# IlzeAmandaA/VAE-GP-ODE

Measured on AMD Instinct MI355X. Metric: latent_trajectories_per_sec, higher is better.
Workload: dtype f32; 1 GPU; configs[1]: ode1 DF q=6 M=100 S=256 T=16 batch=256; step = full ELBO training step (encoder, GP draw, rk4 rollout, decoder, ELBO, backward, Adam), L=1; global_batch=256, mc_draws=1, solver=rk4 (3/8 rule), parallelism=dp1, hip_graph=True, graph_scope=whole, gp_side_stream=True, batchnorm=per-process statistics

## Files before the change

vae-gp-ode_amd/csrc/conv_bwd_v2.hpp:

```cpp
#pragma once
#include "conv_mfma.hpp"

namespace gp {

template <class L> struct BdV2 {
  using PL = BwdDataPolicy<L, L::CI>;
  static constexpr int KC = L::CO, NC = L::CI, KK = L::K * L::K;
  static constexpr int NCT = NC / 16;
  static constexpr int NKS = KK * (KC / 4);
  static constexpr int NPX = L::HI * L::HI;
  static constexpr int SRC = KC * L::HO * L::HO;
  static constexpr int PS = PL::PS, HP = PL::HP, IMG = KC * PS;
  static constexpr int NBUF = 3, NCW = 8, NTHR = 768, NLT = NTHR - 64 * NCW;
  static constexpr int TPW = 2;
  static constexpr int WIN = 16 * 4 * TPW;
  static constexpr int PF = 2;
  static_assert(NCT * 4 == NCW, "the two consumers of a SIMD split the output channels");
  static_assert(KC % 4 == 0 && L::HO % 4 == 0 && SRC % 4 == 0, "float4 rows of the source");
  static_assert(WIN <= NPX, "a window touches at most two images");
  static constexpr int koff(int s) { return (s / (KC / 4)) / L::K * HP + (s / (KC / 4)) % L::K + (s % (KC / 4)) * 4 * PS; }
  static_assert(4 * koff(NKS - 1) < 65536, "operand offsets fit the ds_read immediate");
  static constexpr size_t lds_bytes() { return sizeof(float) * (size_t)NBUF * IMG; }
};

template <class E, int NT>
__device__ __forceinline__ void bdv2_tiles(const float* __restrict__ s_buf, const int (&base)[E::TPW], const float (&wr)[E::NKS],
                                           f32x4 (&acc)[E::TPW]) {
  float bf[E::PF + 1][NT];
  auto fetch = [&](auto sc) {
    constexpr int s = decltype(sc)::value;
#pragma unroll
    for (int t = 0; t < NT; ++t) bf[s % (E::PF + 1)][t] = s_buf[base[t] + E::koff(s)];
  };
#pragma unroll
  for (int t = 0; t < NT; ++t) acc[t] = f32x4{0.f, 0.f, 0.f, 0.f};
  static_for<E::PF>([&](auto sc) { fetch(sc); });
  static_for<E::NKS>([&](auto sc) {
    constexpr int s = decltype(sc)::value;
    if constexpr (s + E::PF < E::NKS) fetch(std::integral_constant<int, s + E::PF>{});
    __builtin_amdgcn_sched_barrier(0);
#pragma unroll
    for (int t = 0; t < NT; ++t) acc[t] = __builtin_amdgcn_mfma_f32_16x16x4f32(wr[s], bf[s % (E::PF + 1)][t], acc[t], 0, 0, 0);
    __builtin_amdgcn_sched_barrier(0);
  });
}

template <class L>
__global__ __launch_bounds__(768) void k_conv_bwd_data_v2(const float* __restrict__ gy, const float* __restrict__ w, float* __restrict__ gx,
                                                          int B) {
  using E = BdV2<L>;
  using PL = typename E::PL;
  constexpr int KC = E::KC, NC = E::NC, KK = E::KK, NPX = E::NPX, IMG = E::IMG, PS = E::PS, HP = E::HP, WIN = E::WIN, NKS = E::NKS;
  constexpr int HO = L::HO, P = L::P, NLT = E::NLT;
  float* s_buf = igemm_smem;
  const int tid = threadIdx.x, lane = tid & 63, wave = __builtin_amdgcn_readfirstlane(tid >> 6);
  const int nit = ((int)blockIdx.x < B) ? (B - 1 - (int)blockIdx.x) / (int)gridDim.x + 1 : 0;
  const int npx = nit * NPX, nwin = (npx + WIN - 1) / WIN;
  auto last_img = [&](int i) { return min(nit - 1, (i * WIN + WIN - 1) / NPX); };

  for (int e = tid; e < E::NBUF * IMG / 4; e += E::NTHR) reinterpret_cast<float4*>(s_buf)[e] = float4{0.f, 0.f, 0.f, 0.f};
  __syncthreads();

  if (wave >= E::NCW) {
    __builtin_amdgcn_s_setprio(3);
    const int lt = tid - 64 * E::NCW;
    constexpr int N4 = E::SRC / 4, NLD = (N4 + NLT - 1) / NLT;
    auto stage = [&](int j) __attribute__((always_inline)) {
      const float4* src = reinterpret_cast<const float4*>(gy) + (size_t)((int)blockIdx.x + j * (int)gridDim.x) * N4;
      float* buf = s_buf + (j % E::NBUF) * IMG;
      float4 v[NLD];
#pragma unroll
      for (int i = 0; i < NLD; ++i) v[i] = src[min(lt + NLT * i, N4 - 1)];
#pragma unroll
      for (int i = 0; i < NLD; ++i) {
        const int f = lt + NLT * i;
        const int pl = (4 * f) / (HO * HO), q = (4 * f) % (HO * HO), row = q / HO, col = q % HO;
        float* d = buf + pl * PS + (row + P) * HP + col + P;
        if (f < N4) { d[0] = v[i].x; d[1] = v[i].y; d[2] = v[i].z; d[3] = v[i].w; }
      }
    };
    if (nit > 0) stage(0);
    __syncthreads();
    for (int i = 0; i < nwin; ++i) {
      if (i + 1 < nwin && last_img(i + 1) > last_img(i)) stage(last_img(i + 1));
      __syncthreads();
    }
    return;
  }

  const int lr = lane & 15, lk = lane >> 4, ct = wave >> 2, sm = wave & 3;
  float wr[NKS];
#pragma unroll
  for (int s = 0; s < NKS; ++s) wr[s] = w[((size_t)(16 * ct + lr) * KC + 4 * (s % (KC / 4)) + lk) * KK + s / (KC / 4)];
  __syncthreads();
  for (int i = 0; i < nwin; ++i) {
    const int t0 = i * WIN + 16 * sm;
    int base[E::TPW], mm[E::TPW];
#pragma unroll
    for (int t = 0; t < E::TPW; ++t) {
      mm[t] = t0 + 64 * t + lr;
      const int m = min(mm[t], npx - 1);
      const int j = m / NPX, p = m - j * NPX;
      base[t] = (j % E::NBUF) * IMG + lk * PS + PL::template C<0>::pix_addr(p);
    }
    f32x4 acc[E::TPW];
    int nt = 0;
    if (t0 + 64 < npx) { bdv2_tiles<E, 2>(s_buf, base, wr, acc); nt = 2; }
    else if (t0 < npx) { bdv2_tiles<E, 1>(s_buf, base, wr, acc); nt = 1; }
#pragma unroll
    for (int t = 0; t < E::TPW; ++t) {
      if (t < nt && mm[t] < npx) {
        const int j = mm[t] / NPX, p = mm[t] - j * NPX;
        float* o = gx + ((size_t)((int)blockIdx.x + j * (int)gridDim.x) * NC + 16 * ct + 4 * lk) * NPX + p;
#pragma unroll
        for (int r = 0; r < 4; ++r) o[(size_t)r * NPX] = acc[t][r];
      }
    }
    __syncthreads();
  }
}

}
```

vae-gp-ode_amd/csrc/vae_conv_tiled.hip:

```cpp
#include <hip/hip_runtime.h>
#include <cstdlib>
#include <cstdint>
#include "gp_launch.hpp"
#include <type_traits>
#include "conv_layers.hpp"
#include "conv_mfma.hpp"
#include "conv_dec10_mfma.hpp"
#include "conv_dec1_mfma.hpp"
#include "conv_dec4_mfma.hpp"

namespace gp {



extern __shared__ __attribute__((aligned(16))) float tsm[];

template <class L, int IPB>
__global__ __launch_bounds__(256) void k_convT_fwd(const float* __restrict__ x, const float* __restrict__ w,
                                                    const float* __restrict__ bias, float* __restrict__ y, int B) {
  constexpr int CI = L::CI, CO = L::CO, HI = L::HI, HO = L::HO, HP = L::HP, K = L::K, S = L::S, P = L::P, PL = L::PL;
  constexpr int CPT = CO % 16 == 0 ? 16 : 8;
  static_assert(CO % CPT == 0, "8 or 16 output channels per thread");
  constexpr int NG = CO / CPT;
  constexpr int IMG = CI * HP * HP;
  float* s_img = tsm;
  float* s_w = tsm + IPB * IMG;
  const int tid = threadIdx.x;
  const int b0 = blockIdx.x * IPB;
  const int nimg = min(IPB, B - b0);
  for (int e = tid; e < IPB * IMG; e += 256) {
    const int im = e / IMG, r = e % IMG, ci = r / (HP * HP), yy = (r / HP) % HP - PL, xx = r % HP - PL;
    float v = 0.f;
    if (im < nimg && yy >= 0 && yy < HI && xx >= 0 && xx < HI) v = x[(((size_t)(b0 + im) * CI + ci) * HI + yy) * HI + xx];
    s_img[e] = v;
  }
  for (int cls = 0; cls < S * S; ++cls) {
    const int py = cls / S, px = cls % S;
    const int nty = (K - py + S - 1) / S, ntx = (K - px + S - 1) / S;
    __syncthreads();
    for (int e = tid; e < nty * ntx * CI * CO; e += 256) {
      const int co = e % CO, ci = (e / CO) % CI, tap = e / (CO * CI);
      const int ky = py + S * (tap / ntx), kx = px + S * (tap % ntx);
      s_w[e] = w[(((size_t)ci * CO + co) * K + ky) * K + kx];
    }
    __syncthreads();
    const int qy0 = (P - py + S - 1 > 0) ? (P - py + S - 1) / S : 0, qx0 = (P - px + S - 1 > 0) ? (P - px + S - 1) / S : 0;
    const int ny = (HO - 1 + P - py) / S - qy0 + 1, nx = (HO - 1 + P - px) / S - qx0 + 1;
    const int items = nimg * ny * nx * NG;
    for (int it = tid; it < items; it += 256) {
      const int g = it % NG, p = (it / NG) % (ny * nx), im = it / (NG * ny * nx);
      const int qy = qy0 + p / nx, qx = qx0 + p % nx;
      float acc[CPT];
#pragma unroll
      for (int c = 0; c < CPT; ++c) acc[c] = bias ? bias[g * CPT + c] : 0.f;
      const float* img = s_img + im * IMG;
      for (int ty = 0; ty < nty; ++ty) {
        for (int tx = 0; tx < ntx; ++tx) {
          const float* ip = img + (qy - ty + PL) * HP + (qx - tx + PL);
          const float4* wp = reinterpret_cast<const float4*>(s_w + ((ty * ntx + tx) * CI) * CO + g * CPT);
#pragma unroll 4
          for (int ci = 0; ci < CI; ++ci) {
            const float v = ip[ci * HP * HP];
#pragma unroll
            for (int q = 0; q < CPT / 4; ++q) {
              const float4 wq = wp[ci * (CO / 4) + q];
              acc[4 * q] = fmaf(v, wq.x, acc[4 * q]); acc[4 * q + 1] = fmaf(v, wq.y, acc[4 * q + 1]);
              acc[4 * q + 2] = fmaf(v, wq.z, acc[4 * q + 2]); acc[4 * q + 3] = fmaf(v, wq.w, acc[4 * q + 3]);
            }
          }
        }
      }
      const int oy = S * qy + py - P, ox = S * qx + px - P;
      float* yp = y + (((size_t)(b0 + im) * CO + g * CPT) * HO + oy) * HO + ox;
#pragma unroll
      for (int c = 0; c < CPT; ++c) yp[(size_t)c * HO * HO] = acc[c];
    }
  }
}


template <class L, int IPB, int COC>
__global__ __launch_bounds__(256) void k_convT_bwd_data(const float* __restrict__ gy, const float* __restrict__ w,
                                                         float* __restrict__ gx, int B) {
  constexpr int CI = L::CI, CO = L::CO, HI = L::HI, HO = L::HO, GPD = L::GP_, K = L::K, S = L::S, P = L::P, KK = K * K;
  static_assert(CI % 16 == 0 && CO % COC == 0, "blocking");
  constexpr int NG = CI / 16;
  constexpr int IMG = CO * GPD * GPD;
  float* s_img = tsm;
  float* s_w = tsm + IPB * IMG;
  const int tid = threadIdx.x;
  const int b0 = blockIdx.x * IPB;
  const int nimg = min(IPB, B - b0);
  for (int e = tid; e < IPB * IMG; e += 256) {
    const int im = e / IMG, r = e % IMG, co = r / (GPD * GPD), yy = (r / GPD) % GPD - P, xx = r % GPD - P;
    float v = 0.f;
    if (im < nimg && yy >= 0 && yy < HO && xx >= 0 && xx < HO) v = gy[(((size_t)(b0 + im) * CO + co) * HO + yy) * HO + xx];
    s_img[e] = v;
  }
  const int items = nimg * HI * HI * NG;
  constexpr int MAXIT = (IPB * HI * HI * NG + 255) / 256;
  float acc[MAXIT][16];
#pragma unroll
  for (int r = 0; r < MAXIT; ++r)
#pragma unroll
    for (int c = 0; c < 16; ++c) acc[r][c] = 0.f;
  for (int c0 = 0; c0 < CO; c0 += COC) {
    __syncthreads();
    for (int e = tid; e < COC * KK * CI; e += 256) {
      const int ci = e % CI, tap = (e / CI) % KK, co = c0 + e / (CI * KK);
      s_w[e] = w[((size_t)ci * CO + co) * KK + tap];
    }
    __syncthreads();
#pragma unroll
    for (int r = 0; r < MAXIT; ++r) {
      const int it = tid + 256 * r;
      if (it < items) {
        const int g = it % NG, p = (it / NG) % (HI * HI), im = it / (NG * HI * HI);
        const int iy = p / HI, ix = p % HI;
        const float* img = s_img + im * IMG + (c0 * GPD + S * iy) * GPD + S * ix;
        for (int co = 0; co < COC; ++co) {
#pragma unroll
          for (int ky = 0; ky < K; ++ky) {
#pragma unroll
            for (int kx = 0; kx < K; ++kx) {
              const float v = img[(co * GPD + ky) * GPD + kx];
              const float4* wp = reinterpret_cast<const float4*>(s_w + ((co * KK + ky * K + kx) * CI) + g * 16);
              const float4 w0 = wp[0], w1 = wp[1], w2 = wp[2], w3 = wp[3];
              float* a = acc[r];
              a[0] = fmaf(v, w0.x, a[0]); a[1] = fmaf(v, w0.y, a[1]); a[2] = fmaf(v, w0.z, a[2]); a[3] = fmaf(v, w0.w, a[3]);
              a[4] = fmaf(v, w1.x, a[4]); a[5] = fmaf(v, w1.y, a[5]); a[6] = fmaf(v, w1.z, a[6]); a[7] = fmaf(v, w1.w, a[7]);
              a[8] = fmaf(v, w2.x, a[8]); a[9] = fmaf(v, w2.y, a[9]); a[10] = fmaf(v, w2.z, a[10]); a[11] = fmaf(v, w2.w, a[11]);
              a[12] = fmaf(v, w3.x, a[12]); a[13] = fmaf(v, w3.y, a[13]); a[14] = fmaf(v, w3.z, a[14]); a[15] = fmaf(v, w3.w, a[15]);
            }
          }
        }
      }
    }
  }
#pragma unroll
  for (int r = 0; r < MAXIT; ++r) {
    const int it = tid + 256 * r;
    if (it < items) {
      const int g = it % NG, p = (it / NG) % (HI * HI), im = it / (NG * HI * HI);
      float* gp = gx + (((size_t)(b0 + im) * CI + g * 16) * HI * HI) + p;
#pragma unroll
      for (int c = 0; c < 16; ++c) gp[(size_t)c * HI * HI] = acc[r][c];
    }
  }
}

template <class L, int COW>
__global__ __launch_bounds__(256) void k_convT_wgrad(const float* __restrict__ x, const float* __restrict__ gy,
                                                      float* __restrict__ part, int B, int b_per_split) {
  constexpr int CI = L::CI, CO = L::CO, HI = L::HI, HO = L::HO, GPD = L::GP_, K = L::K, S = L::S, P = L::P, KK = K * K;
  constexpr int NQ = COW / 4;
  constexpr int NT = CI * NQ;
  constexpr int PSPLIT = 256 / NT;
  static_assert(NT <= 256 && 256 % NT == 0, "thread mapping");
  float* s_x = tsm;
  float* s_g = tsm + HI * HI * CI;
  const int tid = threadIdx.x;
  const int ci = tid % CI, q = (tid / CI) % NQ, ps = tid / NT;
  const int co0 = blockIdx.y * COW;
  const int b0 = blockIdx.x * b_per_split, b1 = min(B, b0 + b_per_split);
  float acc[KK][4];
#pragma unroll
  for (int t = 0; t < KK; ++t) { acc[t][0] = 0.f; acc[t][1] = 0.f; acc[t][2] = 0.f; acc[t][3] = 0.f; }
  for (int b = b0; b < b1; ++b) {
    __syncthreads();
    for (int e = tid; e < HI * HI * CI; e += 256) {
      const int c = e % CI, p = e / CI;
      s_x[e] = x[((size_t)b * CI + c) * HI * HI + p];
    }
    for (int e = tid; e < GPD * GPD * COW; e += 256) {
      const int c = e % COW, xx = (e / COW) % GPD - P, yy = e / (COW * GPD) - P;
      float v = 0.f;
      if (yy >= 0 && yy < HO && xx >= 0 && xx < HO) v = gy[(((size_t)b * CO + co0 + c) * HO + yy) * HO + xx];
      s_g[e] = v;
    }
    __syncthreads();
    for (int p = ps; p < HI * HI; p += PSPLIT) {
      const int iy = p / HI, ix = p % HI;
      const float xv = s_x[p * CI + ci];
      const float* gp = s_g + ((S * iy) * GPD + S * ix) * COW + q * 4;
#pragma unroll
      for (int ky = 0; ky < K; ++ky) {
#pragma unroll
        for (int kx = 0; kx < K; ++kx) {
          const float4 g4 = *reinterpret_cast<const float4*>(gp + (ky * GPD + kx) * COW);
          float* a = acc[ky * K + kx];
          a[0] = fmaf(xv, g4.x, a[0]); a[1] = fmaf(xv, g4.y, a[1]); a[2] = fmaf(xv, g4.z, a[2]); a[3] = fmaf(xv, g4.w, a[3]);
        }
      }
    }
  }
  __syncthreads();
  float* s_red = tsm;
  if (PSPLIT > 1) {
#pragma unroll
    for (int t = 0; t < KK; ++t)
#pragma unroll
      for (int c = 0; c < 4; ++c) s_red[((size_t)ps * NT + (tid % NT)) * (KK * 4) + t * 4 + c] = acc[t][c];
    __syncthreads();
  }
  if (ps == 0) {
    float* out = part + (size_t)blockIdx.x * CI * CO * KK;
#pragma unroll
    for (int t = 0; t < KK; ++t)
#pragma unroll
      for (int c = 0; c < 4; ++c) {
        float v = acc[t][c];
        if (PSPLIT > 1)
          for (int sp = 1; sp < PSPLIT; ++sp) v += s_red[((size_t)sp * NT + (tid % NT)) * (KK * 4) + t * 4 + c];
        out[((size_t)ci * CO + co0 + q * 4 + c) * KK + t] = v;
      }
  }
}


template <int IPB>
__global__ __launch_bounds__(256) void k_dec10_fwd(const float* __restrict__ x, const float* __restrict__ w,
                                                    const float* __restrict__ bias, float* __restrict__ y, int B) {
  constexpr int CI = 16, H = 28, WP = 32, IMG = CI * WP * WP;
  float* s_img = tsm;
  float* s_w = tsm + IPB * IMG;
  const int tid = threadIdx.x;
  const int b0 = blockIdx.x * IPB;
  const int nimg = min(IPB, B - b0);
  for (int e = tid; e < IPB * IMG; e += 256) {
    const int im = e / IMG, r = e % IMG, ci = r / (WP * WP), yy = (r / WP) % WP - 2, xx = r % WP - 2;
    float v = 0.f;
    if (im < nimg && yy >= 0 && yy < H && xx >= 0 && xx < H) v = x[(((size_t)(b0 + im) * CI + ci) * H + yy) * H + xx];
    s_img[e] = v;
  }
  for (int e = tid; e < CI * 5 * 8; e += 256) {
    const int kx = e % 8, ky = (e / 8) % 5, ci = e / 40;
    s_w[e] = kx < 5 ? w[(size_t)ci * 25 + ky * 5 + kx] : 0.f;
  }
  __syncthreads();
  const float bv = bias ? bias[0] : 0.f;
  const int items = nimg * H * 7;
  for (int it = tid; it < items; it += 256) {
    const int seg = it % 7, oy = (it / 7) % H, im = it / (7 * H);
    const int ox0 = seg * 4;
    float acc[4] = {bv, bv, bv, bv};
    const float* img = s_img + im * IMG;
#pragma unroll 2
    for (int ci = 0; ci < CI; ++ci) {
#pragma unroll
      for (int ky = 0; ky < 5; ++ky) {
        const float4* rp = reinterpret_cast<const float4*>(img + (ci * WP + (oy + 4 - ky)) * WP + ox0);
        const float4 a = rp[0], b = rp[1];
        const float v[8] = {a.x, a.y, a.z, a.w, b.x, b.y, b.z, b.w};
        const float4 w4 = *reinterpret_cast<const float4*>(s_w + (ci * 5 + ky) * 8);
        const float w5 = s_w[(ci * 5 + ky) * 8 + 4];
        const float wk[5] = {w4.x, w4.y, w4.z, w4.w, w5};
#pragma unroll
        for (int j = 0; j < 4; ++j)
#pragma unroll
          for (int kx = 0; kx < 5; ++kx) acc[j] = fmaf(v[j + 4 - kx], wk[kx], acc[j]);
      }
    }
    *reinterpret_cast<float4*>(y + ((size_t)(b0 + im) * H + oy) * H + ox0) = make_float4(acc[0], acc[1], acc[2], acc[3]);
  }
}

__global__ __launch_bounds__(256) void k_dec10_wgrad(const float* __restrict__ x, const float* __restrict__ gy,
                                                      float* __restrict__ part, int B, int b_per_split) {
  constexpr int CI = 16, H = 28, NP = H * H, XS = NP + 1, GW = 32;
  float* s_x = tsm;
  float* s_g = tsm + CI * XS;
  const int tid = threadIdx.x, ci = tid & 15, pl = tid >> 4;
  const int b0 = blockIdx.x * b_per_split, b1 = min(B, b0 + b_per_split);
  float acc[25];
#pragma unroll
  for (int t = 0; t < 25; ++t) acc[t] = 0.f;
  for (int b = b0; b < b1; ++b) {
    __syncthreads();
    for (int e = tid; e < CI * NP; e += 256) s_x[(e / NP) * XS + e % NP] = x[(size_t)b * CI * NP + e];
    for (int e = tid; e < GW * GW; e += 256) {
      const int yy = e / GW - 2, xx = e % GW - 2;
      s_g[e] = (yy >= 0 && yy < H && xx >= 0 && xx < H) ? gy[(size_t)b * NP + yy * H + xx] : 0.f;
    }
    __syncthreads();
    for (int p = pl; p < NP; p += 16) {
      const int iy = p / H, ix = p % H;
      const float xv = s_x[ci * XS + p];
      const float* gp = s_g + iy * GW + ix;
#pragma unroll
      for (int ky = 0; ky < 5; ++ky)
#pragma unroll
        for (int kx = 0; kx < 5; ++kx) acc[ky * 5 + kx] = fmaf(xv, gp[ky * GW + kx], acc[ky * 5 + kx]);
    }
  }
  __syncthreads();
  float* s_red = tsm;
#pragma unroll
  for (int t = 0; t < 25; ++t) s_red[(pl * 16 + ci) * 25 + t] = acc[t];
  __syncthreads();
  for (int e = tid; e < CI * 25; e += 256) {
    float v = 0.f;
    for (int l = 0; l < 16; ++l) v += s_red[l * 400 + e];
    part[(size_t)blockIdx.x * 400 + e] = v;
  }
}

__global__ void k_sum_splits_t(const float* __restrict__ part, int nsplit, size_t n, float* __restrict__ out) {
  const size_t e = (size_t)blockIdx.x * blockDim.x + threadIdx.x;
  if (e >= n) return;
  float acc = 0.f;
  for (int s = 0; s < nsplit; ++s) acc += part[(size_t)s * n + e];
  out[e] = acc;
}

template <class L> static bool matches(int Ci_conv, int Co_conv, int H, int Ho, int K, int S, int P) {
  return Ci_conv == L::CO && Co_conv == L::CI && H == L::HO && Ho == L::HI && K == L::K && S == L::S && P == L::P;
}

static bool use_mfma() {
  static int v = -1;
  if (v < 0) { const char* e = getenv("GPODE_CONV_VALU"); v = (e && e[0] == '1') ? 0 : 1; }
  return v == 1;
}

constexpr int kSinkMaxWg = 512;

template <class PL, int IPB, int TG, int NCJ, bool PAIR = false, int NTHR = 512, bool DB = false, bool STATS = false>
static int launch_igemm(const float* x, const float* w, const float* bias, float* y, int B, hipStream_t st, const char* what,
                        const float* in_bn = nullptr, const BnSink* sink = nullptr) {
  constexpr size_t lds = igemm_lds_bytes<PL, IPB, DB, STATS>();
  static_assert(lds <= (NTHR >= 512 ? 160 : 80) * 1024, "LDS budget");
  auto km = k_conv_igemm<PL, IPB, TG, NCJ, PAIR, NTHR, DB, STATS>;
  if (set_max_lds((const void*)km, lds)) return 1;
  const int ngroups = (B + IPB - 1) / IPB;
  const int cap = num_cus() * (NTHR >= 512 ? 1 : 2);
  if (STATS && cap > kSinkMaxWg) return set_error("%s: more workgroups than the statistics scratch holds", what);
  hipLaunchKernelGGL(km, ngroups < cap ? ngroups : cap, NTHR, lds, st, x, w, bias, y, B, in_bn, STATS ? *sink : BnSink{});
  return check_launch(what);
}

template <class L, int IPB, int IPBM, int COS>
static int launch_T1(const float* x, const float* w, const float* bias, float* y, int B, hipStream_t st, const float* in_bn,
                     const BnSink* sink = nullptr) {
  constexpr int MAXTAPS = ((L::K + L::S - 1) / L::S) * ((L::K + L::S - 1) / L::S);
  const size_t lds = sizeof(float) * ((size_t)IPB * L::CI * L::HP * L::HP + (size_t)MAXTAPS * L::CI * L::CO);
  if (use_mfma() && (reinterpret_cast<uintptr_t>(x) & 15) == 0) {
    constexpr int TG = COS >= 64 ? 1 : (COS >= 32 ? 2 : 4);
    constexpr bool PAIR = L::S == 2 && (L::HO % 2 == 0) && (L::P % 2 == 1);
    if constexpr (std::is_same<L, Dec7>::value) {
      static const bool db = [] { const char* e = getenv("GPODE_DEC7_FWD_DB"); return e && e[0] == '1'; }();
      if (db) return launch_igemm<FwdPolicy<L, COS>, 1, TG, COS / 16, PAIR, 512, true>(x, w, bias, y, B, st, "convT_fwd_mfma", in_bn);
    }
    if (sink) return launch_igemm<FwdPolicy<L, COS>, IPBM, TG, COS / 16, PAIR, 512, false, true>(x, w, bias, y, B, st, "convT_fwd_mfma_stats", in_bn, sink);
    return launch_igemm<FwdPolicy<L, COS>, IPBM, TG, COS / 16, PAIR>(x, w, bias, y, B, st, "convT_fwd_mfma", in_bn);
  }
  if (sink) return set_error("convT forward with output statistics needs the matrix-core path (16-byte aligned input, GPODE_CONV_VALU unset)");
  if (in_bn) return set_error("convT forward with a fused BatchNorm input needs the matrix-core path (16-byte aligned input, GPODE_CONV_VALU unset)");
  auto kern = k_convT_fwd<L, IPB>;
  if (set_max_lds((const void*)kern, lds)) return 1;
  hipLaunchKernelGGL(kern, (B + IPB - 1) / IPB, 256, lds, st, x, w, bias, y, B);
  return check_launch("convT_fwd_tiled");
}

template <class L, int IPB, int COC, int IPBM, int CIS, int TG, int NCJ, int NTHR = 512>
static int launch_T2(const float* gy, const float* w, float* gx, int B, hipStream_t st) {
  if constexpr (IPBM > 0) {
    if (use_mfma() && (reinterpret_cast<uintptr_t>(gy) & 15) == 0)
      return launch_igemm<BwdDataPolicy<L, CIS>, IPBM, TG, NCJ, false, NTHR>(gy, w, nullptr, gx, B, st, "convT_bwd_data_mfma");
  }
  const size_t lds = sizeof(float) * ((size_t)IPB * L::CO * L::GP_ * L::GP_ + (size_t)COC * L::K * L::K * L::CI);
  auto kern = k_convT_bwd_data<L, IPB, COC>;
  if (set_max_lds((const void*)kern, lds)) return 1;
  hipLaunchKernelGGL(kern, (B + IPB - 1) / IPB, 256, lds, st, gy, w, gx, B);
  return check_launch("convT_bwd_data_tiled");
}

template <class L, int IPBM, int WM, int WN, int WT, bool PIPE>
static int launch_wgrad_mfma(const float* x, const float* gy, float* gw, float* scratch, int B, hipStream_t st, const float* in_bn) {
  constexpr int NTHR = WM * WN * WT * 64;
  constexpr size_t ldsm = wgrad_lds_bytes<L, IPBM>();
  static_assert(ldsm <= (NTHR == 512 ? 160 : 80) * 1024, "LDS budget");
  auto km = k_convT_wgrad_mfma<L, IPBM, WM, WN, WT, PIPE, false, NTHR>;
  auto kb = k_convT_wgrad_mfma<L, IPBM, WM, WN, WT, PIPE, true, NTHR>;
  if (set_max_lds((const void*)km, ldsm) || set_max_lds((const void*)kb, ldsm)) return 1;
  const int ngroups = (B + IPBM - 1) / IPBM;
  const int cap = num_cus() * (512 / NTHR);
  const int nwg = ngroups < cap ? ngroups : cap;
  if (in_bn) hipLaunchKernelGGL(kb, nwg, NTHR, ldsm, st, x, gy, scratch, B, in_bn);
  else hipLaunchKernelGGL(km, nwg, NTHR, ldsm, st, x, gy, scratch, B, in_bn);
  const size_t n = (size_t)L::CI * L::CO * L::K * L::K;
  if (reduce_job(RedJob{scratch, gw, nwg, (int)n, 1, L::CI / 16, L::CO / 16, L::K * L::K}, st)) return 1;
  return check_launch("convT_wgrad_mfma");
}

int wgrad_v2_dec7(const float* x, const float* gy, float* gw, float* scratch, int B, hipStream_t st, const float* in_bn);
int wgrad_v2_dec4(const float* x, const float* gy, float* gw, float* scratch, int B, hipStream_t st, const float* in_bn);
static bool wgrad_v2_enabled() {
  static const bool off = [] { const char* e = getenv("GPODE_WGRAD_V1"); return e && e[0] == '1'; }();
  return !off && use_mfma();
}

template <class L, int COW, int IPBM, int WM, int WN, int WT, bool PIPE>
static int launch_T3(const float* x, const float* gy, float* gw, float* scratch, int B, hipStream_t st, const float* in_bn) {
  if (use_mfma() && ((reinterpret_cast<uintptr_t>(x) | reinterpret_cast<uintptr_t>(gy)) & 15) == 0)
    return launch_wgrad_mfma<L, IPBM, WM, WN, WT, PIPE>(x, gy, gw, scratch, B, st, in_bn);
  if (in_bn) return set_error("convT weight gradient with a fused BatchNorm input needs the matrix-core path");
  constexpr int NT = L::CI * (COW / 4), PSPLIT = 256 / NT, KK = L::K * L::K;
  size_t fl = (size_t)L::HI * L::HI * L::CI + (size_t)L::GP_ * L::GP_ * COW;
  const size_t red = PSPLIT > 1 ? (size_t)PSPLIT * NT * KK * 4 : 0;
  if (red > fl) fl = red;
  const size_t lds = sizeof(float) * fl;
  int nsplit = B < 256 ? B : 256;
  const int bps = (B + nsplit - 1) / nsplit;
  nsplit = (B + bps - 1) / bps;
  auto kern = k_convT_wgrad<L, COW>;
  if (set_max_lds((const void*)kern, lds)) return 1;
  hipLaunchKernelGGL(kern, dim3(nsplit, L::CO / COW), 256, lds, st, x, gy, scratch, B, bps);
  const size_t n = (size_t)L::CI * L::CO * KK;
  if (reduce_job(RedJob{scratch, gw, nsplit, (int)n, 0, 0, 0, 0}, st)) return 1;
  return check_launch("convT_wgrad_tiled");
}


int tiled_bwd_data(const float* gy, const float* w, const float* bias, float* gx, int B, int Ci, int H, int W, int Co, int K, int S,
                   int P, int Ho, int Wo, const float* in_bn, hipStream_t st, const BnSink* sink) {
  if (H != W || Ho != Wo) return -1;
  if (sink && !(use_mfma() && (matches<Dec7>(Ci, Co, H, Ho, K, S, P) || matches<Dec4>(Ci, Co, H, Ho, K, S, P) ||
                               (matches<Dec1>(Ci, Co, H, Ho, K, S, P) && !in_bn))))
    return set_error("gpode_convT_fwd_stats: no specialisation for this geometry");
  if (matches<Dec7>(Ci, Co, H, Ho, K, S, P)) return launch_T1<Dec7, 3, 2, 16>(gy, w, bias, gx, B, st, in_bn, sink);
  if (matches<Dec4>(Ci, Co, H, Ho, K, S, P)) {
    static const int tapcols = [] { const char* e = getenv("GPODE_DEC4_TAPCOLS"); return e ? (e[0] == '1' ? 1 : 0) : -1; }();
    if ((tapcols == 1 || (tapcols < 0 && B <= 4 * num_cus())) && use_mfma()) {
      const size_t lds = sizeof(float) * (dec4::NPI * dec4::TLD + 4 * dec4::CI + (sink ? 2 * dec4::CO * dec4::NPO : 0));
      if (set_max_lds((const void*)dec4::k_fwd<true>, lds) || set_max_lds((const void*)dec4::k_fwd<false>, lds) ||
          set_max_lds((const void*)dec4::k_fwd<true, true>, lds) || set_max_lds((const void*)dec4::k_fwd<false, true>, lds)) return 1;
      const int nwg = B < num_cus() ? B : num_cus();
      const BnSink sk = sink ? *sink : BnSink{};
      if (sink && in_bn) hipLaunchKernelGGL((dec4::k_fwd<true, true>), nwg, 512, lds, st, gy, w, bias, gx, B, in_bn, sk);
      else if (sink) hipLaunchKernelGGL((dec4::k_fwd<false, true>), nwg, 512, lds, st, gy, w, bias, gx, B, in_bn, sk);
      else if (in_bn) hipLaunchKernelGGL((dec4::k_fwd<true>), nwg, 512, lds, st, gy, w, bias, gx, B, in_bn, sk);
      else hipLaunchKernelGGL((dec4::k_fwd<false>), nwg, 512, lds, st, gy, w, bias, gx, B, in_bn, sk);
      return check_launch("dec4_fwd_tapcols");
    }
    return launch_T1<Dec4, 3, 2, 16>(gy, w, bias, gx, B, st, in_bn, sink);
  }
  if (matches<Dec1>(Ci, Co, H, Ho, K, S, P)) {
    static const bool old = [] { const char* e = getenv("GPODE_DEC1_ENGINE"); return e && e[0] == '1'; }();
    if (!in_bn && use_mfma() && (!old || sink)) {
      const size_t lds = sizeof(float) * 2 * dec1::NPI * dec1::TLD;
      if (set_max_lds((const void*)dec1::k_fwd<false>, lds) || set_max_lds((const void*)dec1::k_fwd<true>, lds)) return 1;
      const int cap = 2 * num_cus();
      if (sink) hipLaunchKernelGGL(dec1::k_fwd<true>, B < cap ? B : cap, 256, lds, st, gy, w, bias, gx, B, *sink);
      else hipLaunchKernelGGL(dec1::k_fwd<false>, B < cap ? B : cap, 256, lds, st, gy, w, bias, gx, B, BnSink{});
      return check_launch("dec1_fwd_mfma");
    }
    return launch_T1<Dec1, 8, 8, 64>(gy, w, bias, gx, B, st, in_bn);
  }
  if (matches<Enc3>(Ci, Co, H, Ho, K, S, P) && !in_bn && B >= 96) {
    constexpr int IPB = 2;
    constexpr int MAXTAPS = ((Enc3::K + Enc3::S - 1) / Enc3::S) * ((Enc3::K + Enc3::S - 1) / Enc3::S);
    const size_t lds = sizeof(float) * ((size_t)IPB * Enc3::CI * Enc3::HP * Enc3::HP + (size_t)MAXTAPS * Enc3::CI * Enc3::CO);
    auto kern = k_convT_fwd<Enc3, IPB>;
    if (set_max_lds((const void*)kern, lds)) return 1;
    hipLaunchKernelGGL(kern, (B + IPB - 1) / IPB, 256, lds, st, gy, w, bias, gx, B);
    return check_launch("enc_conv3_bwd_data_tiled");
  }
  if (matches<Enc6>(Ci, Co, H, Ho, K, S, P) && use_mfma() && (reinterpret_cast<uintptr_t>(gy) & 15) == 0)
  {
    static const bool ipb8 = [] { const char* e = getenv("GPODE_ENC6_IPB8"); return e && e[0] == '1'; }();
    if (!ipb8 && B < 4 * num_cus()) return launch_igemm<FwdPolicy<Enc6, 16>, 2, 4, 1>(gy, w, bias, gx, B, st, "enc_conv6_bwd_data_mfma", in_bn);
    return launch_igemm<FwdPolicy<Enc6, 16>, 8, 4, 1>(gy, w, bias, gx, B, st, "enc_conv6_bwd_data_mfma", in_bn);
  }
  if (matches<Dec10>(Ci, Co, H, Ho, K, S, P)) {
    if (use_mfma()) {
      const size_t ldsm = sizeof(float) * dec10::KK * dec10::PST;
      if (set_max_lds((const void*)dec10::k_fwd<true>, ldsm) || set_max_lds((const void*)dec10::k_fwd<false>, ldsm)) return 1;
      if (in_bn) hipLaunchKernelGGL(dec10::k_fwd<true>, B < num_cus() ? B : num_cus(), 512, ldsm, st, gy, w, bias, gx, B, in_bn);
      else hipLaunchKernelGGL(dec10::k_fwd<false>, B < num_cus() ? B : num_cus(), 512, ldsm, st, gy, w, bias, gx, B, in_bn);
      return check_launch("dec10_fwd_mfma");
    }
    constexpr int IPB = 2;
    const size_t lds = sizeof(float) * ((size_t)IPB * 16 * 32 * 32 + 16 * 5 * 8);
    auto kern = k_dec10_fwd<IPB>;
    if (set_max_lds((const void*)kern, lds)) return 1;
    hipLaunchKernelGGL(kern, (B + IPB - 1) / IPB, 256, lds, st, gy, w, bias, gx, B);
    return check_launch("dec10_fwd");
  }
  return -1;
}

int conv_v2_dec7_bwd_data(const float* gy, const float* w, float* gx, int B, hipStream_t st);
static bool conv_v2_enabled() {
  static const bool off = [] { const char* e = getenv("GPODE_CONV_V1"); return e && e[0] == '1'; }();
  return !off && use_mfma();
}

int tiled_fwd(const float* x, const float* w, const float* bias, float* y, int B, int Ci, int H, int W, int Co, int K, int S, int P,
              int Ho, int Wo, hipStream_t st) {
  if (H != W || Ho != Wo) return -1;
  if (use_mfma() && (reinterpret_cast<uintptr_t>(x) & 15) == 0) {
    if (matches<Enc3>(Ci, Co, H, Ho, K, S, P)) return launch_igemm<BwdDataPolicy<Enc3, 16>, 4, 4, 1>(x, w, bias, y, B, st, "enc_conv3_fwd_mfma");
    if (matches<Enc6>(Ci, Co, H, Ho, K, S, P)) return launch_igemm<BwdDataPolicy<Enc6, 32>, 8, 1, 2>(x, w, bias, y, B, st, "enc_conv6_fwd_mfma");
  }
  if (bias) return -1;
  if (matches<Dec7>(Ci, Co, H, Ho, K, S, P)) {
    if (conv_v2_enabled() && (reinterpret_cast<uintptr_t>(x) & 15) == 0) return conv_v2_dec7_bwd_data(x, w, y, B, st);
    return launch_T2<Dec7, 2, 8, 1, 16, 2, 1, 256>(x, w, y, B, st);
  }
  if (matches<Dec4>(Ci, Co, H, Ho, K, S, P)) {
    static const bool alt = [] { const char* e = getenv("GPODE_DEC4_BWD_3IMG"); return e && e[0] == '1'; }();
    if (alt) return launch_T2<Dec4, 3, 8, 3, 16, 1, 1>(x, w, y, B, st);
    return launch_T2<Dec4, 3, 8, 2, 32, 1, 1>(x, w, y, B, st);
  }
  if (matches<Dec1>(Ci, Co, H, Ho, K, S, P)) {
    static const bool old = [] { const char* e = getenv("GPODE_DEC1_ENGINE"); return e && e[0] == '1'; }();
    if (use_mfma() && !old && (reinterpret_cast<uintptr_t>(x) & 15) == 0) {
      const size_t lds = sizeof(float) * (2 * dec1::GYF + 4 * dec1::NPI * 33);
      const int cap = 2 * num_cus();
      hipLaunchKernelGGL(dec1::k_bwd_data, B < cap ? B : cap, 256, lds, st, x, w, y, B);
      return check_launch("dec1_bwd_data_mfma");
    }
    return launch_T2<Dec1, 8, 32, 6, 32, 1, 1>(x, w, y, B, st);
  }

  if (matches<Dec10>(Ci, Co, H, Ho, K, S, P)) {
    if (use_mfma() && (reinterpret_cast<uintptr_t>(x) & 15) == 0) {
      constexpr int IPB = 8;
      const size_t ldsm = sizeof(float) * IPB * dec10::PLANE;
      const int ngroups = (B + IPB - 1) / IPB;
      hipLaunchKernelGGL(dec10::k_bwd_data<IPB>, ngroups < num_cus() ? ngroups : num_cus(), 512, ldsm, st, x, w, y, B);
      return check_launch("dec10_bwd_data_mfma");
    }
    return launch_T2<Dec10, 1, 1, 0, 16, 1, 1>(x, w, y, B, st);
  }
  return -1;
}

constexpr int kDec10BnMaxWg = 512;
int dec10_bn_scratch_floats() { return 2 * kDec10BnMaxWg * dec10::CI * 2; }

__global__ __launch_bounds__(512) void k_dec10_parts_reduce(const float* __restrict__ part, int nsplit, float* __restrict__ out, int stride2) {
  __shared__ float sA[dec10::CI], sB[dec10::CI];
  dec10::reduce_parts(part, nsplit, sA, sB);
  __syncthreads();
  const int tid = threadIdx.x;
  if (stride2) { if (tid < 2 * dec10::CI) out[tid] = (tid & 1 ? sB : sA)[tid >> 1]; }
  else if (tid < dec10::CI) out[tid] = sA[tid];
}

template <int IPB, int MODE, bool WGRAD = false, typename... A>
static int launch_dec10_bn(int B, hipStream_t st, A... args) {
  const size_t lds = sizeof(float) * ((size_t)IPB * dec10::PLANE + 8 * 4 * dec10::CI * 2 + 2 * dec10::CI + (WGRAD ? 8 * dec10::CI * 32 : 0));
  auto kern = dec10::k_bwd_data_bn<IPB, MODE, WGRAD>;
  if (set_max_lds((const void*)kern, lds)) return 1;
  const int ngroups = (B + IPB - 1) / IPB, cap = 2 * num_cus() < kDec10BnMaxWg ? 2 * num_cus() : kDec10BnMaxWg;
  hipLaunchKernelGGL(kern, ngroups < cap ? ngroups : cap, 512, lds, st, args...);
  return 0;
}
static int dec10_bn_nwg(int B, int& ipb) {
  ipb = B >= 4 * num_cus() ? 4 : 2;
  const int ngroups = (B + ipb - 1) / ipb, cap = 2 * num_cus() < kDec10BnMaxWg ? 2 * num_cus() : kDec10BnMaxWg;
  return ngroups < cap ? ngroups : cap;
}

int dec10_bn_wgrad_scratch_floats() { return kDec10BnMaxWg * dec10::CI * dec10::KK + kDec10BnMaxWg; }
int dec10_bn_bwd_sums(const float* c, const float* gy, const float* w, const float* gamma, const float* beta, const float* mean,
                      const float* invstd, float* sums, int B, float* scratch, hipStream_t st, float* gw, float* wscratch, float* gbias) {
  if (((reinterpret_cast<uintptr_t>(gy) | reinterpret_cast<uintptr_t>(c)) & 15) != 0) return set_error("gpode_dec10_bn_bwd_sums: c / gy must be 16-byte aligned");
  if (gw && !wscratch) return set_error("gpode_dec10_bn_bwd_sums_wgrad: scratch for the weight-gradient partials missing");
  int ipb;
  const int nwg = dec10_bn_nwg(B, ipb);
  float* np_ = nullptr;
  const float* cnp = nullptr;
  int rc;
  if (gw) {
    float* part_b = gbias ? wscratch + (size_t)kDec10BnMaxWg * dec10::CI * dec10::KK : nullptr;
    if (ipb == 4) rc = launch_dec10_bn<4, 0, true>(B, st, gy, w, c, gamma, beta, mean, invstd, B, scratch, 0, 0.f, cnp, cnp, 0, np_, np_, np_, np_, wscratch, part_b);
    else rc = launch_dec10_bn<2, 0, true>(B, st, gy, w, c, gamma, beta, mean, invstd, B, scratch, 0, 0.f, cnp, cnp, 0, np_, np_, np_, np_, wscratch, part_b);
    if (!rc) {
      const RedJob jobs[2] = {RedJob{wscratch, gw, nwg, dec10::CI * dec10::KK, 0, 0, 0, 0}, RedJob{part_b, gbias, nwg, 1, 0, 0, 0, 0}};
      if (reduce_jobs(jobs, gbias ? 2 : 1, st)) return 1;
    }
  } else if (ipb == 4) rc = launch_dec10_bn<4, 0>(B, st, gy, w, c, gamma, beta, mean, invstd, B, scratch, 0, 0.f, cnp, cnp, 0, np_, np_, np_, np_, np_, np_);
  else rc = launch_dec10_bn<2, 0>(B, st, gy, w, c, gamma, beta, mean, invstd, B, scratch, 0, 0.f, cnp, cnp, 0, np_, np_, np_, np_, np_, np_);
  if (rc) return rc;
  if (sums) hipLaunchKernelGGL(k_dec10_parts_reduce, 1, 512, 0, st, scratch, nwg, sums, 1);
  return check_launch("dec10_bn_bwd_sums");
}

int dec10_bn_bwd_apply(const float* c, const float* gy, const float* w, const float* gamma, const float* beta, const float* mean,
                       const float* invstd, const float* gathered, const float* wts, int W, float count_all, float* gc, float* ggamma,
                       float* gbeta, float* gc_chansum, int B, float* scratch, hipStream_t st) {
  if (((reinterpret_cast<uintptr_t>(gy) | reinterpret_cast<uintptr_t>(c) | reinterpret_cast<uintptr_t>(gc)) & 15) != 0)
    return set_error("gpode_dec10_bn_bwd_apply: c / gy / gc must be 16-byte aligned");
  if (gathered && (W < 1 || !wts)) return set_error("gpode_dec10_bn_bwd_apply: gathered sums need their weights");
  int ipb;
  const int nwg = dec10_bn_nwg(B, ipb);
  float* part_gx = gc_chansum ? scratch + (size_t)kDec10BnMaxWg * dec10::CI * 2 : nullptr;
  const float count = gathered ? count_all : (float)B * dec10::NP;
  int rc;
  if (ipb == 4) rc = launch_dec10_bn<4, 1>(B, st, gy, w, c, gamma, beta, mean, invstd, B, scratch, nwg, count, gathered, wts, W, ggamma, gbeta, gc, part_gx, (float*)nullptr, (float*)nullptr);
  else rc = launch_dec10_bn<2, 1>(B, st, gy, w, c, gamma, beta, mean, invstd, B, scratch, nwg, count, gathered, wts, W, ggamma, gbeta, gc, part_gx, (float*)nullptr, (float*)nullptr);
  if (rc) return rc;
  if (gc_chansum && reduce_job(RedJob{part_gx, gc_chansum, nwg, dec10::CI, 2, 0, 0, 0}, st)) return 1;
  return check_launch("dec10_bn_bwd_apply");
}

int tiled_bwd_weight(const float* x, const float* gy, float* gw, float* scratch, int B, int Ci, int H, int W, int Co, int K, int S,
                     int P, int Ho, int Wo, const float* in_bn, hipStream_t st) {
  if (H != W || Ho != Wo) return -1;
  const bool aligned = ((reinterpret_cast<uintptr_t>(x) | reinterpret_cast<uintptr_t>(gy)) & 15) == 0;
  if (matches<Dec7>(Ci, Co, H, Ho, K, S, P)) {
    if (wgrad_v2_enabled() && aligned) return wgrad_v2_dec7(gy, x, gw, scratch, B, st, in_bn);
    return launch_T3<Dec7, 16, 2, 1, 1, 8, true>(gy, x, gw, scratch, B, st, in_bn);
  }
  if (matches<Dec4>(Ci, Co, H, Ho, K, S, P)) {
    if (wgrad_v2_enabled() && aligned) return wgrad_v2_dec4(gy, x, gw, scratch, B, st, in_bn);
    return launch_T3<Dec4, 16, 2, 4, 2, 1, false>(gy, x, gw, scratch, B, st, in_bn);
  }
  if (matches<Dec1>(Ci, Co, H, Ho, K, S, P)) {
    static const bool old = [] { const char* e = getenv("GPODE_DEC1_ENGINE"); return e && e[0] == '1'; }();
    if (!in_bn && use_mfma() && !old && (reinterpret_cast<uintptr_t>(x) & 15) == 0) {
      const size_t lds = sizeof(float) * 2 * dec1::GYF;
      static const int wcap = [] { const char* e = getenv("GPODE_DEC1_WGRAD_WGS"); return e ? atoi(e) : 256; }();
      const int cap = 2 * num_cus() < wcap ? 2 * num_cus() : wcap;
      const int nwg = B < cap ? B : cap;
      hipLaunchKernelGGL(dec1::k_wgrad, nwg, 256, lds, st, gy, x, scratch, B);
      if (reduce_job(RedJob{scratch, gw, nwg, dec1::CI * dec1::NN, 0, 0, 0, 0}, st)) return 1;
      return check_launch("dec1_wgrad_mfma");
    }
    return launch_T3<Dec1, 32, 8, 2, 4, 1, true>(gy, x, gw, scratch, B, st, in_bn);
  }
  if (matches<Enc6>(Ci, Co, H, Ho, K, S, P) && use_mfma() && ((reinterpret_cast<uintptr_t>(x) | reinterpret_cast<uintptr_t>(gy)) & 15) == 0)
    return launch_wgrad_mfma<Enc6, 8, 2, 1, 4, true>(gy, x, gw, scratch, B, st, in_bn);
  if (matches<Dec10>(Ci, Co, H, Ho, K, S, P) && use_mfma() &&
      ((reinterpret_cast<uintptr_t>(x) | reinterpret_cast<uintptr_t>(gy)) & 15) == 0) {
    constexpr int IPB = 1;
    const size_t fl = (size_t)IPB * dec10::PLANE > 8 * 16 * 32 ? (size_t)IPB * dec10::PLANE : 8 * 16 * 32;
    const int ngroups = (B + IPB - 1) / IPB;
    const int nwg = ngroups < num_cus() ? ngroups : num_cus();
    hipLaunchKernelGGL(dec10::k_wgrad<IPB>, nwg, 512, sizeof(float) * fl, st, gy, x, scratch, B, in_bn);
    if (reduce_job(RedJob{scratch, gw, nwg, 400, 0, 0, 0, 0}, st)) return 1;
    return check_launch("dec10_wgrad_mfma");
  }
  if (matches<Dec10>(Ci, Co, H, Ho, K, S, P)) {
    int nsplit = B < 256 ? B : 256;
    const int bps = (B + nsplit - 1) / nsplit;
    nsplit = (B + bps - 1) / bps;
    const size_t lds = sizeof(float) * (16 * 785 + 32 * 32);
    if (set_max_lds((const void*)k_dec10_wgrad, lds)) return 1;
    hipLaunchKernelGGL(k_dec10_wgrad, nsplit, 256, lds, st, gy, x, scratch, B, bps);
    if (reduce_job(RedJob{scratch, gw, nsplit, 400, 0, 0, 0, 0}, st)) return 1;
    return check_launch("dec10_wgrad");
  }
  return -1;
}

}
```

vae-gp-ode_amd/csrc/vae_conv_v2.hip:

```cpp
#include <hip/hip_runtime.h>
#include <cstdint>
#include "gp_launch.hpp"
#include "conv_layers.hpp"
#include "conv_bwd_v2.hpp"

namespace gp {

int conv_v2_dec7_bwd_data(const float* gy, const float* w, float* gx, int B, hipStream_t st) {
  using E = BdV2<Dec7>;
  constexpr size_t lds = E::lds_bytes();
  static_assert(lds <= 160 * 1024, "LDS budget");
  auto km = k_conv_bwd_data_v2<Dec7>;
  if (set_max_lds((const void*)km, lds)) return 1;
  hipLaunchKernelGGL(km, B < num_cus() ? B : num_cus(), E::NTHR, lds, st, gy, w, gx, B);
  return check_launch("conv_v2_dec7_bwd_data");
}

}
```

Baseline: 100,400 trajectories/s.

## Route Dec4 backward-data conv through generalized MFMA producer/consumer v2 kernel

Result: faster. 104,300 trajectories/s (median of 6 runs) (+3.9%).

```diff
diff --git a/vae-gp-ode_amd/csrc/conv_bwd_v2.hpp b/vae-gp-ode_amd/csrc/conv_bwd_v2.hpp
--- a/vae-gp-ode_amd/csrc/conv_bwd_v2.hpp
+++ b/vae-gp-ode_amd/csrc/conv_bwd_v2.hpp
@@ -11,13 +11,19 @@
   static constexpr int NPX = L::HI * L::HI;
   static constexpr int SRC = KC * L::HO * L::HO;
   static constexpr int PS = PL::PS, HP = PL::HP, IMG = KC * PS;
-  static constexpr int NBUF = 3, NCW = 8, NTHR = 768, NLT = NTHR - 64 * NCW;
-  static constexpr int TPW = 2;
-  static constexpr int WIN = 16 * 4 * TPW;
+  static constexpr int CPS = NKS <= 100 ? 2 : 1;
+  static constexpr int NCW = 4 * CPS, NTHR = 64 * (NCW + 4), NLT = NTHR - 64 * NCW;
+  static constexpr int TSPLIT = NCW / NCT;
+  static constexpr int TPW = CPS == 2 ? 2 : 4;
+  static constexpr int WIN = 16 * TSPLIT * TPW;
   static constexpr int PF = 2;
-  static_assert(NCT * 4 == NCW, "the two consumers of a SIMD split the output channels");
-  static_assert(KC % 4 == 0 && L::HO % 4 == 0 && SRC % 4 == 0, "float4 rows of the source");
-  static_assert(WIN <= NPX, "a window touches at most two images");
+  static constexpr int NTMIN = CPS == 2 ? 1 : TPW;
+  static constexpr int NBUF = (2 * WIN - 2) / NPX + 2;
+  static_assert(NCW % NCT == 0 && TSPLIT * NCT == NCW, "the consumers split the ci tiles evenly");
+  static_assert(TPW * (PF + 1) <= 15, "LDS reads in flight within what lgkmcnt counts");
+  static_assert(KC % 4 == 0 && SRC % 4 == 0, "float4 source");
+  static constexpr bool ROW4 = L::HO % 4 == 0;
+  static_assert(ROW4 || L::HO * L::HO <= NLT, "producer offset table");
   static constexpr int koff(int s) { return (s / (KC / 4)) / L::K * HP + (s / (KC / 4)) % L::K + (s % (KC / 4)) * 4 * PS; }
   static_assert(4 * koff(NKS - 1) < 65536, "operand offsets fit the ds_read immediate");
   static constexpr size_t lds_bytes() { return sizeof(float) * (size_t)NBUF * IMG; }
@@ -45,70 +51,99 @@
   });
 }
 
+template <class E, int NT>
+__device__ __forceinline__ void bdv2_window(int nt, const float* __restrict__ s_buf, const int (&base)[E::TPW], const float (&wr)[E::NKS],
+                                            f32x4 (&acc)[E::TPW]) {
+  if constexpr (NT > E::NTMIN) {
+    if (nt < NT) { bdv2_window<E, NT - 1>(nt, s_buf, base, wr, acc); return; }
+  }
+  bdv2_tiles<E, NT>(s_buf, base, wr, acc);
+}
+
 template <class L>
-__global__ __launch_bounds__(768) void k_conv_bwd_data_v2(const float* __restrict__ gy, const float* __restrict__ w, float* __restrict__ gx,
-                                                          int B) {
+__global__ __launch_bounds__(BdV2<L>::NTHR) void k_conv_bwd_data_v2(const float* __restrict__ gy, const float* __restrict__ w,
+                                                                    float* __restrict__ gx, int B) {
   using E = BdV2<L>;
   using PL = typename E::PL;
   constexpr int KC = E::KC, NC = E::NC, KK = E::KK, NPX = E::NPX, IMG = E::IMG, PS = E::PS, HP = E::HP, WIN = E::WIN, NKS = E::NKS;
-  constexpr int HO = L::HO, P = L::P, NLT = E::NLT;
+  constexpr int HO = L::HO, P = L::P, NLT = E::NLT, NBUF = E::NBUF, TPW = E::TPW, TSPLIT = E::TSPLIT;
   float* s_buf = igemm_smem;
   const int tid = threadIdx.x, lane = tid & 63, wave = __builtin_amdgcn_readfirstlane(tid >> 6);
   const int nit = ((int)blockIdx.x < B) ? (B - 1 - (int)blockIdx.x) / (int)gridDim.x + 1 : 0;
   const int npx = nit * NPX, nwin = (npx + WIN - 1) / WIN;
   auto last_img = [&](int i) { return min(nit - 1, (i * WIN + WIN - 1) / NPX); };
 
-  for (int e = tid; e < E::NBUF * IMG / 4; e += E::NTHR) reinterpret_cast<float4*>(s_buf)[e] = float4{0.f, 0.f, 0.f, 0.f};
+  for (int e = tid; e < NBUF * IMG / 4; e += E::NTHR) reinterpret_cast<float4*>(s_buf)[e] = float4{0.f, 0.f, 0.f, 0.f};
   __syncthreads();
 
   if (wave >= E::NCW) {
     __builtin_amdgcn_s_setprio(3);
     const int lt = tid - 64 * E::NCW;
-    constexpr int N4 = E::SRC / 4, NLD = (N4 + NLT - 1) / NLT;
+    constexpr int N4 = E::SRC / 4;
+    int otab[4];
+#pragma unroll
+    for (int k = 0; k < 4; ++k) {
+      const int e = 4 * min(lt, HO * HO - 1) + k, pl = e / (HO * HO), q = e % (HO * HO);
+      otab[k] = pl * PS + (q / HO + P) * HP + q % HO + P;
+    }
     auto stage = [&](int j) __attribute__((always_inline)) {
       const float4* src = reinterpret_cast<const float4*>(gy) + (size_t)((int)blockIdx.x + j * (int)gridDim.x) * N4;
-      float* buf = s_buf + (j % E::NBUF) * IMG;
-      float4 v[NLD];
+      float* buf = s_buf + (j % NBUF) * IMG;
+      if constexpr (E::ROW4) {
+        constexpr int NLD = (N4 + NLT - 1) / NLT;
+        float4 v[NLD];
 #pragma unroll
-      for (int i = 0; i < NLD; ++i) v[i] = src[min(lt + NLT * i, N4 - 1)];
+        for (int i = 0; i < NLD; ++i) v[i] = src[min(lt + NLT * i, N4 - 1)];
 #pragma unroll
-      for (int i = 0; i < NLD; ++i) {
-        const int f = lt + NLT * i;
-        const int pl = (4 * f) / (HO * HO), q = (4 * f) % (HO * HO), row = q / HO, col = q % HO;
-        float* d = buf + pl * PS + (row + P) * HP + col + P;
-        if (f < N4) { d[0] = v[i].x; d[1] = v[i].y; d[2] = v[i].z; d[3] = v[i].w; }
+        for (int i = 0; i < NLD; ++i) {
+          const int f = lt + NLT * i;
+          const int pl = (4 * f) / (HO * HO), q = (4 * f) % (HO * HO), row = q / HO, col = q % HO;
+          float* d = buf + pl * PS + (row + P) * HP + col + P;
+          if (f < N4) { d[0] = v[i].x; d[1] = v[i].y; d[2] = v[i].z; d[3] = v[i].w; }
+        }
+      } else if (lt < HO * HO) {
+        float4 v[KC / 4];
+#pragma unroll
+        for (int g = 0; g < KC / 4; ++g) v[g] = src[g * HO * HO + lt];
+#pragma unroll
+        for (int g = 0; g < KC / 4; ++g) {
+          float* d = buf + 4 * g * PS;
+          d[otab[0]] = v[g].x; d[otab[1]] = v[g].y; d[otab[2]] = v[g].z; d[otab[3]] = v[g].w;
+        }
       }
     };
-    if (nit > 0) stage(0);
+    int staged = -1;
+    if (nit > 0)
+      for (; staged < last_img(0); ) stage(++staged);
     __syncthreads();
     for (int i = 0; i < nwin; ++i) {
-      if (i + 1 < nwin && last_img(i + 1) > last_img(i)) stage(last_img(i + 1));
+      if (i + 1 < nwin)
+        for (const int j1 = last_img(i + 1); staged < j1; ) stage(++staged);
       __syncthreads();
     }
     return;
   }
 
-  const int lr = lane & 15, lk = lane >> 4, ct = wave >> 2, sm = wave & 3;
+  const int lr = lane & 15, lk = lane >> 4, ct = wave / TSPLIT, sm = wave % TSPLIT;
   float wr[NKS];
 #pragma unroll
   for (int s = 0; s < NKS; ++s) wr[s] = w[((size_t)(16 * ct + lr) * KC + 4 * (s % (KC / 4)) + lk) * KK + s / (KC / 4)];
   __syncthreads();
   for (int i = 0; i < nwin; ++i) {
     const int t0 = i * WIN + 16 * sm;
-    int base[E::TPW], mm[E::TPW];
+    int base[TPW], mm[TPW];
 #pragma unroll
-    for (int t = 0; t < E::TPW; ++t) {
-      mm[t] = t0 + 64 * t + lr;
+    for (int t = 0; t < TPW; ++t) {
+      mm[t] = t0 + 16 * TSPLIT * t + lr;
       const int m = min(mm[t], npx - 1);
       const int j = m / NPX, p = m - j * NPX;
-      base[t] = (j % E::NBUF) * IMG + lk * PS + PL::template C<0>::pix_addr(p);
+      base[t] = (j % NBUF) * IMG + lk * PS + PL::template C<0>::pix_addr(p);
     }
-    f32x4 acc[E::TPW];
-    int nt = 0;
-    if (t0 + 64 < npx) { bdv2_tiles<E, 2>(s_buf, base, wr, acc); nt = 2; }
-    else if (t0 < npx) { bdv2_tiles<E, 1>(s_buf, base, wr, acc); nt = 1; }
+    f32x4 acc[TPW];
+    const int nt = t0 < npx ? min(TPW, (npx - t0 + 16 * TSPLIT - 1) / (16 * TSPLIT)) : 0;
+    if (nt > 0) bdv2_window<E, TPW>(nt, s_buf, base, wr, acc);
 #pragma unroll
-    for (int t = 0; t < E::TPW; ++t) {
+    for (int t = 0; t < TPW; ++t) {
       if (t < nt && mm[t] < npx) {
         const int j = mm[t] / NPX, p = mm[t] - j * NPX;
         float* o = gx + ((size_t)((int)blockIdx.x + j * (int)gridDim.x) * NC + 16 * ct + 4 * lk) * NPX + p;
diff --git a/vae-gp-ode_amd/csrc/vae_conv_tiled.hip b/vae-gp-ode_amd/csrc/vae_conv_tiled.hip
--- a/vae-gp-ode_amd/csrc/vae_conv_tiled.hip
+++ b/vae-gp-ode_amd/csrc/vae_conv_tiled.hip
@@ -491,6 +491,7 @@
 }
 
 int conv_v2_dec7_bwd_data(const float* gy, const float* w, float* gx, int B, hipStream_t st);
+int conv_v2_dec4_bwd_data(const float* gy, const float* w, float* gx, int B, hipStream_t st);
 static bool conv_v2_enabled() {
   static const bool off = [] { const char* e = getenv("GPODE_CONV_V1"); return e && e[0] == '1'; }();
   return !off && use_mfma();
@@ -509,6 +510,7 @@
     return launch_T2<Dec7, 2, 8, 1, 16, 2, 1, 256>(x, w, y, B, st);
   }
   if (matches<Dec4>(Ci, Co, H, Ho, K, S, P)) {
+    if (conv_v2_enabled() && (reinterpret_cast<uintptr_t>(x) & 15) == 0) return conv_v2_dec4_bwd_data(x, w, y, B, st);
     static const bool alt = [] { const char* e = getenv("GPODE_DEC4_BWD_3IMG"); return e && e[0] == '1'; }();
     if (alt) return launch_T2<Dec4, 3, 8, 3, 16, 1, 1>(x, w, y, B, st);
     return launch_T2<Dec4, 3, 8, 2, 32, 1, 1>(x, w, y, B, st);
diff --git a/vae-gp-ode_amd/csrc/vae_conv_v2.hip b/vae-gp-ode_amd/csrc/vae_conv_v2.hip
--- a/vae-gp-ode_amd/csrc/vae_conv_v2.hip
+++ b/vae-gp-ode_amd/csrc/vae_conv_v2.hip
@@ -6,14 +6,22 @@
 
 namespace gp {
 
-int conv_v2_dec7_bwd_data(const float* gy, const float* w, float* gx, int B, hipStream_t st) {
-  using E = BdV2<Dec7>;
+template <class L> static int launch_bwd_data_v2(const float* gy, const float* w, float* gx, int B, hipStream_t st, const char* what) {
+  using E = BdV2<L>;
   constexpr size_t lds = E::lds_bytes();
   static_assert(lds <= 160 * 1024, "LDS budget");
-  auto km = k_conv_bwd_data_v2<Dec7>;
+  auto km = k_conv_bwd_data_v2<L>;
   if (set_max_lds((const void*)km, lds)) return 1;
   hipLaunchKernelGGL(km, B < num_cus() ? B : num_cus(), E::NTHR, lds, st, gy, w, gx, B);
-  return check_launch("conv_v2_dec7_bwd_data");
+  return check_launch(what);
+}
+
+int conv_v2_dec7_bwd_data(const float* gy, const float* w, float* gx, int B, hipStream_t st) {
+  return launch_bwd_data_v2<Dec7>(gy, w, gx, B, st, "conv_v2_dec7_bwd_data");
+}
+
+int conv_v2_dec4_bwd_data(const float* gy, const float* w, float* gx, int B, hipStream_t st) {
+  return launch_bwd_data_v2<Dec4>(gy, w, gx, B, st, "conv_v2_dec4_bwd_data");
 }
 
 }
```
